# dtarb/TauDEM

Measured on AMD Instinct MI355X. Metric: Mcells/s (PitRemove->D8FlowDir->AreaD8 pipeline), higher is better.
Workload: dtype f32

## Files before the change

### taudem_amd/csrc/d8flowdir.hip

```cpp
#include <cstring>

#include "context.hpp"
#include "device_common.hpp"
#include "flats.hpp"

namespace {

using namespace tdxk;

constexpr int SLOPE_ROWS = 16;

constexpr int SLOPE_COLS = 62;
using flatmask_t = uint32_t;
template <int SLOPE_SEG>
__global__ __launch_bounds__(256) void d8_slope_kernel(const float* __restrict__ Z, int nx, int ny, int y_own0, int y_own1, float nodata,
                                                       const double* __restrict__ fact, int16_t* __restrict__ P,
                                                       float* __restrict__ SD8, flatmask_t* __restrict__ flatbits, int nbx, int xmap) {
    using tilek::lane_left;
    using tilek::lane_right;
    const int bx = tdxk::xcd_block_x(nbx, xmap);
    if (bx < 0) return;
    const int lx = threadIdx.x & 63;
    const int x = bx * SLOPE_COLS - 1 + lx;
    const int band = __builtin_amdgcn_readfirstlane(int(blockIdx.y) * 4 + int(threadIdx.x >> 6));
// ... 76 lines not shown
    for (unsigned b0 = 0; b0 < nblocks; b0 += 1024) {
        const unsigned i = b0 + threadIdx.x;
        const unsigned long long own = i < nblocks ? blocksum[i] : 0u;
        unsigned long long v = own;
#pragma unroll
        for (int off = 1; off < 64; off <<= 1) {
            const unsigned long long t = __shfl_up(v, off, 64);
            if (int(threadIdx.x & 63) >= off) v += t;
        }
        if ((threadIdx.x & 63) == 63) sw[threadIdx.x >> 6] = v;
        __syncthreads();
        unsigned long long wave_off = carry;
        for (unsigned w = 0; w < (threadIdx.x >> 6); w++) wave_off += sw[w];
        if (i < nblocks) blocksum[i] = unsigned(wave_off + v - own);
        __syncthreads();
        if (threadIdx.x == 1023) carry = wave_off + v;
        __syncthreads();
    }
    if (threadIdx.x == 0) *total = carry;
}
__global__ __launch_bounds__(256) void flat_list_kernel(const flatmask_t* __restrict__ bits, size_t nmasks, int nx, int y_own0, int seg, const unsigned* __restrict__ blockoff,
                                                        uint32_t* __restrict__ list) {
    constexpr int NCH = FLATQ_PER_BLOCK / 256;
    const size_t base = size_t(blockIdx.x) * FLATQ_PER_BLOCK + threadIdx.x;
    const int lane = int(threadIdx.x & 63), w = int(threadIdx.x >> 6);
    unsigned mk[NCH];
    __shared__ unsigned scnt[NCH][4];
#pragma unroll
    for (int i = 0; i < NCH; i++) {
        const size_t m = base + size_t(i) * 256;
        mk[i] = m < nmasks ? bits[m] : 0u;
        unsigned c = unsigned(__popc(mk[i]));
#pragma unroll
        for (int off = 32; off >= 1; off >>= 1) c += __shfl_xor(c, off, 64);
        if (lane == 0) scnt[i][w] = c;
    }
    __syncthreads();
    const unsigned long long below = (1ull << lane) - 1ull;
#pragma unroll
    for (int i = 0; i < NCH; i++) {
        unsigned any = mk[i];
#pragma unroll
        for (int off = 32; off >= 1; off >>= 1) any |= __shfl_xor(any, off, 64);
        if (!any) continue;
        unsigned pos = blockoff[blockIdx.x];
        for (int j = 0; j < i; j++) pos += scnt[j][0] + scnt[j][1] + scnt[j][2] + scnt[j][3];
        for (int u = 0; u < w; u++) pos += scnt[i][u];
        const size_t m = base + size_t(i) * 256, mc = m < nmasks ? m : nmasks - 1;
        const unsigned band = unsigned(mc / size_t(nx)), x = unsigned(mc - size_t(band) * size_t(nx));
        const size_t c0 = size_t(y_own0 + int(band) * seg) * size_t(nx) + size_t(x);
        for (unsigned rows = any; rows; rows &= rows - 1u) {
            const int r = __ffs(int(rows)) - 1;
            const bool mine = (mk[i] >> r) & 1u;
            const unsigned long long b = __ballot(mine);
            if (mine) list[pos + unsigned(__popcll(b & below))] = uint32_t(c0 + size_t(r) * size_t(nx));
            pos += unsigned(__popcll(b));
        }
    }
}

__device__ __forceinline__ bool dont_cross_d8(const int16_t* __restrict__ P, size_t c, int nx, int k) {
    switch (k) {
        case 2: return P[c + 1] == 4 || P[c - nx] == 8;
        case 4: return P[c - nx] == 6 || P[c - 1] == 2;
        case 6: return P[c + nx] == 4 || P[c - 1] == 8;
        case 8: return P[c + 1] == 6 || P[c + nx] == 2;
        default: return false;
    }
}

struct D8Codes {
    using Raw = int;
    const int16_t* P;
    __device__ __forceinline__ int load(size_t o) const { return P[o]; }
    static __device__ __forceinline__ unsigned onehot(int p) { return (1u << min(unsigned(p), 31u)) & 0x1FFu; }
};

struct D8Traits {
    const int16_t* P;
    __device__ __forceinline__ bool dont_cross(size_t c, int nx, int k) const { return dont_cross_d8(P, c, nx, k); }
    __device__ __forceinline__ bool has_direction(size_t n) const { const int16_t v = P[n]; return v > 0 && v < 9; }
};

template <class LV>
__global__ __launch_bounds__(256) void d8_setflow2_kernel(const float* __restrict__ Z, int nx, const double* __restrict__ fact,
                                                          const uint32_t* __restrict__ list, unsigned long long nq,
                                                          const LV* __restrict__ lvl, const LV* __restrict__ rq,
                                                          FlatLevels fl, int16_t* __restrict__ P) {
    const unsigned long long q = (unsigned long long)blockIdx.x * 256 + threadIdx.x;
    if (q >= nq) return;
    const size_t c = list[q];
    const int y = int(c / size_t(nx));
    const double* f = fact + size_t(y) * 9;
    const int e2c = int(flat_elev2<LV>(lvl[c], rq[c], fl));
    const float z0 = Z[c];
    float smax = 0.f;
    int16_t dir = P[c];
    const int order[8] = {1, 3, 5, 7, 2, 4, 6, 8};
    for (int o = 0; o < 8; o++) {
        const int k = order[o];
        const size_t n = size_t(ptrdiff_t(c) + ptrdiff_t(d2(k)) * nx + d1(k));
        if (rq[n] > 0) {
            const int e2n = int(flat_elev2<LV>(lvl[n], rq[n], fl));
            const float slope = (float)(f[k] * (double)(e2c - e2n));
            if (slope > smax) { dir = int16_t(k); smax = slope; }
        } else {
            const float ed = z0 - Z[n];
            if (ed >= 0) { dir = int16_t(k); break; }
        }
    }
    P[c] = dir;
}

__global__ __launch_bounds__(256) void d8_recollect_kernel(const int16_t* __restrict__ P, const uint32_t* __restrict__ list,
                                                           unsigned long long nq, uint32_t* __restrict__ out,
                                                           unsigned long long* __restrict__ counter) {
    const unsigned long long q0 = ((unsigned long long)blockIdx.x * 256 + threadIdx.x) * 8;
    uint32_t keep[8];
    unsigned cnt = 0;
#pragma unroll
    for (int i = 0; i < 8; i++) {
        const unsigned long long q = q0 + (unsigned long long)i;
        if (q < nq) {
            const uint32_t c = list[q];
            if (P[c] == 0) keep[cnt++] = c;
        }
    }
    unsigned long long pos = block_reserve(cnt, counter);
    for (unsigned i = 0; i < cnt; i++) out[pos + i] = keep[i];
}

template <class LV>
__global__ __launch_bounds__(256) void d8_mark_pits_kernel(const uint32_t* __restrict__ list, unsigned long long nq,
                                                           const LV* __restrict__ lvl, int16_t* __restrict__ P) {
    const unsigned long long q = (unsigned long long)blockIdx.x * 256 + threadIdx.x;
    if (q >= nq) return;
    const size_t c = list[q];
    if (lvl[c] == 0) P[c] = TDX_P_NODATA;
}

constexpr int SF2_COLS = 62;
template <class LV>
__global__ __launch_bounds__(256) void d8_setflow2_stream_kernel(const float* __restrict__ Z, int nx, int ny, int y_own0, int y_own1,
                                                                 const double* __restrict__ fact, const LV* __restrict__ lvl,
                                                                 const LV* __restrict__ rq, FlatLevels fl, int16_t* __restrict__ P,
                                                                 uint32_t* __restrict__ qnext, unsigned long long* __restrict__ counter, int nbx, int xmap,
                                                                 LV* __restrict__ lvl_next, LV* __restrict__ rq_next) {
    using tilek::lane_left;
    using tilek::lane_right;
    const int bx = tdxk::xcd_block_x(nbx, xmap);
    if (bx < 0) return;
    const int lx = threadIdx.x & 63;
    const int x = bx * SF2_COLS - 1 + lx;
    const int ybase = __builtin_amdgcn_readfirstlane(y_own0 + blockIdx.y * (4 * SLOPE_ROWS) + (threadIdx.x >> 6) * SLOPE_ROWS);
    const bool mine = lx >= 1 && lx <= SF2_COLS && x < nx;
    const int xc = x < 0 ? 0 : (x >= nx ? nx - 1 : x);
    int16_t p[SLOPE_ROWS];
#pragma unroll
    for (int r = 0; r < SLOPE_ROWS; r++) {
        const int y = ybase + r, yc = y >= ny ? ny - 1 : y;
        p[r] = P[size_t(yc) * size_t(nx) + size_t(xc)];
    }
    unsigned flat = 0;
    unsigned rows0 = 0;
#pragma unroll
    for (int r = 0; r < SLOPE_ROWS; r++) {
        const bool f0 = mine && ybase + r < y_own1 && p[r] == 0;
        if (f0) flat |= 1u << r;
        if (__ballot(f0) != 0ull) rows0 |= 1u << r;
    }
    unsigned keep = 0;
    if (rows0) {
        const unsigned need = rows0 | (rows0 << 1) | (rows0 << 2);
        float z[SLOPE_ROWS + 2];
        int e2[SLOPE_ROWS + 2], rr[SLOPE_ROWS + 2];
#pragma unroll
        for (int j = 0; j < SLOPE_ROWS + 2; j++) {
            z[j] = 0.f; e2[j] = -1; rr[j] = -1;
            if ((need >> j) & 1u) {
                const int y = ybase - 1 + j, yc = y < 0 ? 0 : (y >= ny ? ny - 1 : y);
                const size_t o = size_t(yc) * size_t(nx) + size_t(xc);
                z[j] = Z[o]; e2[j] = lvl[o]; rr[j] = rq[o];
            }
        }
        unsigned pit = 0;
#pragma unroll
        for (int j = 0; j < SLOPE_ROWS + 2; j++) {
            if (e2[j] == 0) pit |= 1u << j;
            e2[j] = int(flat_elev2<LV>(e2[j], rr[j], fl));
        }
#pragma unroll
        for (int r = 0; r < SLOPE_ROWS; r++) {
            if (!((rows0 >> r) & 1u)) continue;
            const int y = ybase + r;
            const float zk[9] = {0.f, lane_right(z[r + 1], 0.f), lane_right(z[r], 0.f), z[r], lane_left(z[r], 0.f), lane_left(z[r + 1], 0.f),
                                 lane_left(z[r + 2], 0.f), z[r + 2], lane_right(z[r + 2], 0.f)};
            const int rk[9] = {0, lane_right(rr[r + 1], -1), lane_right(rr[r], -1), rr[r], lane_left(rr[r], -1), lane_left(rr[r + 1], -1),
                               lane_left(rr[r + 2], -1), rr[r + 2], lane_right(rr[r + 2], -1)};
            const int ek[9] = {0, lane_right(e2[r + 1], 0), lane_right(e2[r], 0), e2[r], lane_left(e2[r], 0), lane_left(e2[r + 1], 0),
                               lane_left(e2[r + 2], 0), e2[r + 2], lane_right(e2[r + 2], 0)};
            if ((flat >> r) & 1u) {
                const double* f = fact + size_t(y) * 9;
                const int e2c = e2[r + 1];
                const float z0 = z[r + 1];
                float smax = 0.f;
                int16_t dir = (fl.has_pits && ((pit >> (r + 1)) & 1u)) ? TDX_P_NODATA : int16_t(0);
                bool done = false;
#define TDX_SF2(K)                                                                     \
    if (!done) {                                                                        \
        const float slope = (float)(f[K] * (double)(e2c - ek[K]));                      \
        const bool marked = rk[K] > 0;                                                  \
        const bool take = marked && slope > smax;                                       \
        const bool stop = !marked && z0 - zk[K] >= 0;                                   \
        dir = (take || stop) ? int16_t(K) : dir;                                        \
        smax = take ? slope : smax;                                                     \
        done = stop;                                                                    \
    }
                TDX_SF2(1) TDX_SF2(3) TDX_SF2(5) TDX_SF2(7) TDX_SF2(2) TDX_SF2(4) TDX_SF2(6) TDX_SF2(8)
#undef TDX_SF2
                P[size_t(y) * size_t(nx) + size_t(x)] = dir;
                if (dir == 0) keep |= 1u << r;
            }
        }
    }
    if (lvl_next != nullptr) {
#pragma unroll
        for (int r = 0; r < SLOPE_ROWS; r++) {
            if (mine && ybase + r < y_own1) {
                const size_t idx = size_t(ybase + r) * size_t(nx) + size_t(x);
                const LV m = ((keep >> r) & 1u) ? LV(0) : LV(-1);
                lvl_next[idx] = m;
                rq_next[idx] = m;
            }
        }
    }
    const unsigned long long pos = block_reserve(unsigned(__popc(keep)), counter);
    const unsigned long long wbase = (unsigned long long)(unsigned(__builtin_amdgcn_readfirstlane(int(unsigned(pos))))) |
                                     ((unsigned long long)(unsigned(__builtin_amdgcn_readfirstlane(int(unsigned(pos >> 32))))) << 32);
    const unsigned long long below = (1ull << lx) - 1ull;
    unsigned rowoff = 0;
#pragma unroll
    for (int r = 0; r < SLOPE_ROWS; r++) {
        const unsigned long long b = __ballot((keep >> r) & 1u);
        if ((keep >> r) & 1u) qnext[wbase + rowoff + unsigned(__popcll(b & below))] = uint32_t(size_t(ybase + r) * size_t(nx) + size_t(x));
        rowoff += unsigned(__popcll(b));
    }
}

}

int tdx_build_fact_table(tdx_context* ctx, int64_t ny, const double* dxc, const double* dyc, double** d_fact_out) {
    static const int hd1[9] = {0, 1, 1, 0, -1, -1, -1, 0, 1};
    static const int hd2[9] = {0, 0, -1, -1, -1, 0, 1, 1, 1};
    const size_t rows = size_t(ny);
    if (ctx->fact_dxc.size() == rows && ctx->fact_dyc.size() == rows && memcmp(ctx->fact_dxc.data(), dxc, rows * 8) == 0 &&
        memcmp(ctx->fact_dyc.data(), dyc, rows * 8) == 0) {
        *d_fact_out = static_cast<double*>(ctx->scratch(TDX_S_FACT, rows * 9 * sizeof(double)));
        return *d_fact_out ? TDX_OK : TDX_ERR_NOMEM;
    }
    ctx->fact_dxc.clear(); ctx->fact_dyc.clear();
    std::vector<double> fact(rows * 9, 0.0);
    for (int64_t m = 0; m < ny; m++)
        for (int k = 1; k <= 8; k++)
            fact[size_t(m) * 9 + size_t(k)] = (double)(1. / sqrt(hd1[k] * hd1[k] * dxc[m] * dxc[m] + hd2[k] * hd2[k] * dyc[m] * dyc[m]));
    double* d_fact = static_cast<double*>(ctx->scratch(TDX_S_FACT, fact.size() * sizeof(double)));
    if (!d_fact) return TDX_ERR_NOMEM;
    TDX_HIP_CHECK(ctx, hipMemcpyAsync(d_fact, fact.data(), fact.size() * sizeof(double), hipMemcpyHostToDevice, ctx->stream));
    TDX_HIP_CHECK(ctx, hipStreamSynchronize(ctx->stream));
    ctx->fact_dxc.assign(dxc, dxc + rows);
    ctx->fact_dyc.assign(dyc, dyc + rows);
    *d_fact_out = d_fact;
    return TDX_OK;
}

template <class LV>
static int d8flowdir_levels(tdx_context* ctx, const Strip& st, float* d_fel, float fel_nodata, const double* dxc, const double* dyc, int16_t* d_p,
                          float* d_sd8, tdx_stats* stats) {
    TDX_HIP_CHECK(ctx, hipSetDevice(ctx->device));
    hipStream_t s = ctx->stream;
    const int inx = st.nx;
    const size_t n = size_t(st.nx) * size_t(st.ny_arr);
    double* d_fact = nullptr;
    int rc = tdx_build_fact_table(ctx, st.ny_arr, dxc, dyc, &d_fact);
    if (rc != TDX_OK) return rc;
    unsigned long long* d_cnt = reinterpret_cast<unsigned long long*>(ctx->d_mail);
    LV* lvl = static_cast<LV*>(ctx->scratch(TDX_S_A, n * sizeof(LV)));
    LV* rq = static_cast<LV*>(ctx->scratch(TDX_S_B, n * sizeof(LV)));
    uint32_t* qlist = static_cast<uint32_t*>(ctx->scratch(TDX_S_C, n * 4));
    if (!lvl || !rq || !qlist) return TDX_ERR_NOMEM;

    ctx->begin_call(stats);
    strip_mark(ctx, st, "d8flowdir");
    ctx->phase = "slope pass";
    rc = strip_exchange<float>(ctx, st, d_fel, fel_nodata);
    if (rc != TDX_OK) return rc;
    TDX_HIP_CHECK(ctx, hipMemsetAsync(d_cnt, 0, 8 * sizeof(unsigned long long), s));
    static const int seg = (getenv("TDX_SLOPE_SEG") && atoi(getenv("TDX_SLOPE_SEG")) == 16) ? 16 : 32;
    const int nband = ((st.y1 - st.y0 + 4 * seg - 1) / (4 * seg)) * 4;
    const size_t nmasks = size_t(nband) * size_t(inx);
    const unsigned nqblocks = unsigned((nmasks + FLATQ_PER_BLOCK - 1) / FLATQ_PER_BLOCK);
    flatmask_t* flatbits = static_cast<flatmask_t*>(ctx->scratch(TDX_S_N, nmasks * sizeof(flatmask_t)));
    unsigned* blocksum = static_cast<unsigned*>(ctx->scratch(TDX_S_O, size_t(nqblocks) * 4));
    if (!flatbits || !blocksum) return TDX_ERR_NOMEM;
    {
        TdxSpan sp(ctx, TDX_K_STENCIL);
        const int nbx = (inx + SLOPE_COLS - 1) / SLOPE_COLS, xmap = tdx_xcd_map() ? 1 : 0;
        dim3 grid(tdx_xcd_grid_x(unsigned(nbx)), unsigned(nband / 4));
        if (seg == 16) hipLaunchKernelGGL(d8_slope_kernel<16>, grid, dim3(256), 0, s, d_fel, inx, st.ny_arr, st.y0, st.y1, fel_nodata, d_fact, d_p, d_sd8, flatbits, nbx, xmap);
        else hipLaunchKernelGGL(d8_slope_kernel<32>, grid, dim3(256), 0, s, d_fel, inx, st.ny_arr, st.y0, st.y1, fel_nodata, d_fact, d_p, d_sd8, flatbits, nbx, xmap);
        if (stats) stats->launches[TDX_K_STENCIL]++;
    }
    {
        TdxSpan sp(ctx, TDX_K_MISC);
        hipLaunchKernelGGL(flat_count_kernel, dim3(nqblocks), dim3(256), 0, s, flatbits, nmasks, blocksum);
        hipLaunchKernelGGL(flat_scan_kernel, dim3(1), dim3(1024), 0, s, blocksum, nqblocks, d_cnt);
    }
    TDX_HIP_CHECK(ctx, hipMemcpyAsync(ctx->h_mail, d_cnt, sizeof(unsigned long long), hipMemcpyDeviceToHost, s));
    TDX_HIP_CHECK(ctx, hipStreamSynchronize(s));
    unsigned long long nq = ctx->h_mail[0];
    int64_t total = int64_t(nq);
    rc = strip_allreduce(ctx, st, &total, 1, TDX_OP_SUM);
    if (rc != TDX_OK) return rc;
    if (stats) { stats->flats_initial = total; stats->flats_left = total; }

    const bool force_list = getenv("TDX_FLATS_LIST") != nullptr;
    const bool have_list = force_list || nq <= n / 16;
    if (total > 0 && nq > 0 && have_list) {
        TdxSpan sp(ctx, TDX_K_MISC);
        hipLaunchKernelGGL(flat_list_kernel, dim3(nqblocks), dim3(256), 0, s, flatbits, nmasks, inx, st.y0, seg, blocksum, qlist);
    }
    if (total > 0) {
        rc = strip_exchange<int16_t>(ctx, st, d_p, TDX_P_NODATA);
        if (rc != TDX_OK) return rc;
        uint32_t* qnext = static_cast<uint32_t*>(ctx->scratch(TDX_S_D, size_t(nq) * 4));
        if (!qnext) return TDX_ERR_NOMEM;
        float* zwork = nullptr;
        const float* zcur = d_fel;
        FlatBuffersT<LV> fbuf{lvl, rq};

        int64_t last = total;
        const int64_t total0 = total;
        bool sparse = false;
        unsigned long long nq_old = 0;
        bool old_list_valid = false;
        LV *lvl_next = nullptr, *rq_next = nullptr;
        bool markers_ready = false;
        for (int iteration = 1;; iteration++) {
            const FlatPhases& ph = flat_phases(iteration);
            ctx->phase = ph.classify;
            FlatLevels fl;
            D8Traits tr{d_p};
            const float* zc = zcur;
            const StreamClassifyFn classify = [&](const tilek::TileGeom& g, uint8_t* fmask, uint8_t* rmask, uint32_t* tile_flags, uint8_t* tile_masked, uint8_t* notfull) {
                const int nbx = (st.nx + flatk::CLS_COLS - 1) / flatk::CLS_COLS;
                const dim3 grid(tdx_xcd_grid_x(unsigned(nbx)), (st.y1 - st.y0 + 4 * flatk::CLS_ROWS - 1) / (4 * flatk::CLS_ROWS));
                hipLaunchKernelGGL((flatk::classify_stream_kernel<LV, D8Codes>), grid, dim3(256), 0, s, zc, D8Codes{d_p}, st.nx, st.ny_arr, st.y0, st.y1, g.tiles_x, lvl, rq, fmask,
                                   rmask, tile_flags, tile_masked, nbx, tdx_xcd_map() ? 1 : 0, notfull);
            };
            if (sparse && markers_ready) {
                std::swap(lvl, lvl_next);
                std::swap(rq, rq_next);
                fbuf = FlatBuffersT<LV>{lvl, rq};
                rc = strip_exchange<LV>(ctx, st, lvl, LV(-1));
                if (rc != TDX_OK) return rc;
                rc = strip_exchange<LV>(ctx, st, rq, LV(-1));
                if (rc != TDX_OK) return rc;
            } else if (sparse) {
                rc = old_list_valid ? flats_reset_markers_after(ctx, st, qnext, nq_old, qlist, nq, lvl, rq) : flats_reset_markers(ctx, st, qlist, nq, lvl, rq);
                if (rc != TDX_OK) return rc;
            }
            markers_ready = false;
            rc = flats_bfs<D8Traits, LV>(ctx, tr, zcur, st, (nq_old == 0 && !have_list) ? nullptr : qlist, nq, fbuf, &fl, stats, sparse ? nullptr : &classify, iteration);
            if (rc != TDX_OK) return rc;
            ctx->phase = ph.directions;
            {
                TdxSpan sp(ctx, TDX_K_FLATDIR);
                unsigned long long* d_next = d_cnt + 4;
                if (nq > n / 32) {
                    const int nbx = (st.nx + SF2_COLS - 1) / SF2_COLS;
                    const dim3 grid(tdx_xcd_grid_x(unsigned(nbx)), (st.y1 - st.y0 + 4 * SLOPE_ROWS - 1) / (4 * SLOPE_ROWS));
                    static const bool no_next = getenv("TDX_FLATS_NO_NEXT_MARKERS") != nullptr;
                    if (!no_next && !lvl_next) {
                        lvl_next = static_cast<LV*>(ctx->scratch(TDX_S_P, n * sizeof(LV)));
                        rq_next = static_cast<LV*>(ctx->scratch(TDX_S_R, n * sizeof(LV)));
                        if (!lvl_next || !rq_next) return TDX_ERR_NOMEM;
                    }
                    hipLaunchKernelGGL((d8_setflow2_stream_kernel<LV>), grid, dim3(256), 0, s, zcur, inx, st.ny_arr, st.y0, st.y1, d_fact, lvl, rq, fl, d_p, qnext,
                                       d_next, nbx, tdx_xcd_map() ? 1 : 0, lvl_next, rq_next);
                    markers_ready = lvl_next != nullptr;
                } else if (nq) {
                    if (fl.has_pits)
                        hipLaunchKernelGGL((d8_mark_pits_kernel<LV>), dim3(tdx_blocks_for(nq, 256)), dim3(256), 0, s, qlist, nq, lvl, d_p);
                    hipLaunchKernelGGL((d8_setflow2_kernel<LV>), dim3(tdx_blocks_for(nq, 256)), dim3(256), 0, s, zcur, inx, d_fact, qlist, nq, lvl, rq, fl, d_p);
                    hipLaunchKernelGGL(d8_recollect_kernel, dim3(tdx_blocks_for(nq, 2048)), dim3(256), 0, s, d_p, qlist, nq, qnext, d_next);
                }
                TDX_HIP_CHECK(ctx, hipMemcpyAsync(ctx->h_mail, d_next, sizeof(unsigned long long), hipMemcpyDeviceToHost, s));
                TDX_HIP_CHECK(ctx, hipStreamSynchronize(s));
                if (stats) stats->launches[TDX_K_FLATDIR] += 2 + (fl.has_pits ? 1 : 0);
            }
            const unsigned long long nleft = ctx->h_mail[0];
            total = int64_t(nleft);
            rc = strip_allreduce(ctx, st, &total, 1, TDX_OP_SUM);
            if (rc != TDX_OK) return rc;
            rc = strip_exchange<int16_t>(ctx, st, d_p, TDX_P_NODATA);
            if (rc != TDX_OK) return rc;
            if (stats) { stats->flat_iterations++; stats->flats_left = total; }
            if (!(total > 0 && total < last)) break;
            ctx->phase = ph.next;
            if (!zwork) {
                zwork = static_cast<float*>(ctx->scratch(TDX_S_I, n * 4));
                if (!zwork) return TDX_ERR_NOMEM;
            }
            static const bool no_sparse = getenv("TDX_FLATS_DENSE") != nullptr;
            sparse = !no_sparse && (total * 8 <= total0 || total <= (int64_t(1) << 20));
            rc = sparse ? flats_overwrite_elevation_sparse(ctx, inx, qnext, nleft, lvl, rq, fl, zwork) : flats_overwrite_elevation(ctx, n, lvl, rq, fl, zwork);
            if (rc != TDX_OK) return rc;
            zcur = zwork;
            old_list_valid = nq_old != 0 || have_list;
            nq_old = nq;
            std::swap(qlist, qnext);
            nq = nleft;
            last = total;
        }
    }
    TDX_HIP_CHECK(ctx, hipGetLastError());
    ctx->end_call();
    return TDX_OK;
}

static int d8flowdir_impl(tdx_context* ctx, const Strip& st, float* d_fel, float fel_nodata, const double* dxc, const double* dyc, int16_t* d_p,
                          float* d_sd8, tdx_stats* stats) {
    int rc = getenv("TDX_LEVELS_INT32") ? TDX_FLATS_TOO_DEEP : d8flowdir_levels<int16_t>(ctx, st, d_fel, fel_nodata, dxc, dyc, d_p, d_sd8, stats);
    if (rc == TDX_FLATS_TOO_DEEP) rc = d8flowdir_levels<int32_t>(ctx, st, d_fel, fel_nodata, dxc, dyc, d_p, d_sd8, stats);
    return rc;
}

static int d8flowdir_check(tdx_context* ctx, const void* fel, const void* p, const void* dxc, const void* dyc, int64_t nx, int64_t ny, int64_t halo, const char* who) {
    if (!ctx || !fel || !p || !dxc || !dyc || nx <= 0 || ny <= 0) return tdx_fail(ctx, TDX_ERR_ARG, who);
    return too_big(nx, ny + halo) ? tdx_fail(ctx, TDX_ERR_ARG, "raster larger than 2^32 cells per device strip") : TDX_OK;
}

extern "C" int tdx_d8flowdir_dev(tdx_context* ctx, const float* d_fel, int64_t nx, int64_t ny, float fel_nodata,
                                 const double* dxc, const double* dyc, int16_t* d_p, float* d_sd8, tdx_stats* stats) {
    if (int rc = d8flowdir_check(ctx, d_fel, d_p, dxc, dyc, nx, ny, 0, "tdx_d8flowdir_dev: bad argument")) return rc;
    return d8flowdir_impl(ctx, strip_single(int(nx), int(ny)), const_cast<float*>(d_fel), fel_nodata, dxc, dyc, d_p, d_sd8, stats);
}

extern "C" int tdx_d8flowdir_strip(tdx_context* ctx, const tdx_comm* comm, float* d_fel, int64_t nx, int64_t ny_local, float fel_nodata,
                                   const double* dxc, const double* dyc, int16_t* d_p, float* d_sd8, tdx_stats* stats) {
    if (int rc = d8flowdir_check(ctx, d_fel, d_p, dxc, dyc, nx, ny_local, 2, "tdx_d8flowdir_strip: bad argument")) return rc;
    return d8flowdir_impl(ctx, strip_from_comm(comm, int(nx), int(ny_local)), d_fel, fel_nodata, dxc, dyc, d_p, d_sd8, stats);
}

extern "C" int tdx_d8flowdir(tdx_context* ctx, const float* fel, int64_t nx, int64_t ny, float fel_nodata,
                             const double* dxc, const double* dyc, int16_t* p, float* sd8, tdx_stats* stats) {
    if (!ctx || !fel || !p || nx <= 0 || ny <= 0) return tdx_fail(ctx, TDX_ERR_ARG, "tdx_d8flowdir: bad argument");
    HostCall h(ctx, nx, ny);
    float* d_z = h.in(TDX_S_IO0, fel);
    int16_t* d_p = h.out(TDX_S_IO1, p);
    float* d_s = h.out(TDX_S_IO2, sd8);
    if (h.error) return h.error;
    return h.finish(tdx_d8flowdir_dev(ctx, d_z, nx, ny, fel_nodata, dxc, dyc, d_p, d_s, stats));
}
```

### taudem_amd/csrc/dinfflowdir.hip

```cpp
#include "context.hpp"
#include "device_common.hpp"
#include "flats.hpp"

namespace {
using namespace tdxk;

#define TDX_PI 3.14159265359

__host__ __device__ constexpr int fI1(int K) { return int((0x1a505u >> (2 * K)) & 3u) - 1; }
__host__ __device__ constexpr int fI2(int K) { return int((0x2a801u >> (2 * K)) & 3u) - 1; }
__host__ __device__ constexpr int fJ1(int K) { return int((0x25059u >> (2 * K)) & 3u) - 1; }
__host__ __device__ constexpr int fJ2(int K) { return int((0x28029u >> (2 * K)) & 3u) - 1; }
__host__ __device__ constexpr bool fID1_is1(int K) { return ((0x132u >> K) & 1u) != 0u; }
__host__ __device__ constexpr double fANGC(int K) { return double(K / 2); }
__host__ __device__ constexpr double fANGF(int K) { return (K & 1) ? 1.0 : -1.0; }
__device__ __forceinline__ double fANGC_rt(int K) { return double(K >> 1); }
__device__ __forceinline__ double fANGF_rt(int K) { return (K & 1) ? 1.0 : -1.0; }
static_assert(fI1(3) == -1 && fI2(5) == 1 && fJ1(4) == -1 && fJ2(8) == 1 && fID1_is1(1) && !fID1_is1(2) && fID1_is1(8), "facet tables");

struct RowGeom { double dx, dy, dd, ad12, ad21; };

__device__ __forceinline__ void vslope(double E0, double E1, double E2, double D1, double D2, double DD, double AD, double& S, double& A) {
    double S1 = 0, S2 = 0;
    if (D1 != 0) S1 = (E0 - E1) / D1;
    if (D2 != 0) S2 = (E1 - E2) / D2;
    if (S2 == 0 && S1 == 0) A = 0;
    else A = atan2(S2, S1);
    if (A < 0.) { A = 0.; S = S1; }
    else if (A > AD) { A = AD; S = (E0 - E2) / DD; }
    else S = sqrt(S1 * S1 + S2 * S2);
}

__device__ __forceinline__ void facet_geom(const RowGeom& g, int K, double& D1, double& D2, double& AD) {
    const bool one = fID1_is1(K);
    D1 = one ? g.dx : g.dy;
    D2 = one ? g.dy : g.dx;
    AD = one ? g.ad12 : g.ad21;
}

template <class T>
__device__ __forceinline__ T sel4(int i, T a0, T a1, T a2, T a3) { return i == 0 ? a0 : (i == 1 ? a1 : (i == 2 ? a2 : a3)); }
__device__ __forceinline__ int facet_cardinal(int K) { return (K & 7) >> 1; }
__device__ __forceinline__ int facet_diagonal(int K) { return (K - 1) >> 1; }

__device__ __forceinline__ double vslope_s(double E0, double E1, double E2, double D1, double D2, double DD, double AD, int* kind, double* s1o, double* s2o) {
    const double S1 = (E0 - E1) / D1, S2 = (E1 - E2) / D2;
    *s1o = S1; *s2o = S2;
    int kd;
    if (S2 == 0 && S1 == 0) kd = 2;
    else if (S2 < 0) kd = 0;
    else if (S2 == 0) kd = S1 > 0 ? 2 : 1;
    else if (S1 <= 0) kd = 1;
    else {
        const double l = S2 * D1, r = S1 * D2;
        if (fabs(l - r) > 1e-9 * (l + r)) kd = l > r ? 1 : 2;
        else kd = atan2(S2, S1) > atan2(D2, D1) ? 1 : 2;
    }
    *kind = kd;
    if (kd == 0) return S1;
    if (kd == 1) return (E0 - E2) / DD;
    return sqrt(S1 * S1 + S2 * S2);
}

constexpr int DSLOPE_ROWS = 16;
__global__ __launch_bounds__(256) void dinf_slope_kernel(const float* __restrict__ Z, int nx, int ny, int y_own0, int y_own1, float nodata,
                                                         const RowGeom* __restrict__ geom, float* __restrict__ ANG,
                                                         float* __restrict__ SLP, unsigned long long* __restrict__ nflat) {
    const int x = blockIdx.x * 64 + (threadIdx.x & 63);
    const int ybase = y_own0 + blockIdx.y * (4 * DSLOPE_ROWS) + (threadIdx.x >> 6) * DSLOPE_ROWS;
    const bool colok = x < nx;
    const int xc = colok ? x : nx - 1, xm = xc > 0 ? xc - 1 : xc, xp = xc < nx - 1 ? xc + 1 : xc;
    auto ldrow = [&](int y, float& a, float& b, float& c) {
        if (y >= 0 && y < ny) {
            const float* r = Z + size_t(y) * size_t(nx);
            a = r[xm]; b = r[xc]; c = r[xp];
        } else { a = b = c = nodata; }
    };
    float n0, n1, n2, c0, c1, c2, s0, s1, s2;
    ldrow(ybase - 1, n0, n1, n2);
    ldrow(ybase, c0, c1, c2);
    unsigned nfl = 0;
#pragma unroll
// ... 36 lines not shown
                }
            }
            ANG[idx] = ang;
            SLP[idx] = slp;
        }
        n0 = c0; n1 = c1; n2 = c2;
        c0 = s0; c1 = s1; c2 = s2;
    }
    (void)block_reserve(nfl, nflat);
}


struct DinfTraits {
    const float* ANG;
    __device__ __forceinline__ bool dont_cross(size_t c, int nx, int k) const {
        switch (k) {
            case 2: return ANG[c + 1] == 4 || ANG[c - nx] == 8;
            case 4: return ANG[c - nx] == 6 || ANG[c - 1] == 2;
            case 6: return ANG[c + nx] == 4 || ANG[c - 1] == 8;
            case 8: return ANG[c + 1] == 6 || ANG[c + nx] == 2;
            default: return false;
        }
    }
    __device__ __forceinline__ bool has_direction(size_t n) const { return ANG[n] >= 0.0f; }
};

__device__ __forceinline__ bool dinf_is_flat(float a) { return !is_nodata_f(a, TDX_ANG_NODATA) && a < 0.0f; }

struct DinfCodes {
    using Raw = float;
    const float* ANG;
    __device__ __forceinline__ float load(size_t o) const { return ANG[o]; }
    static __device__ __forceinline__ unsigned onehot(float a) {
        if (is_nodata_f(a, TDX_ANG_NODATA)) return 0u;
        if (a < 0.0f) return 1u;
        return a == 2.0f ? 1u << 2 : (a == 4.0f ? 1u << 4 : (a == 6.0f ? 1u << 6 : (a == 8.0f ? 1u << 8 : 1u << 1)));
    }
};

template <class LV>
__global__ __launch_bounds__(256) void dinf_collect_flats_kernel(const float* __restrict__ ANG, size_t first, size_t n, LV* __restrict__ lvl,
                                                                 LV* __restrict__ rq, uint32_t* __restrict__ list,
                                                                 unsigned long long* __restrict__ counter) {
    const size_t c0 = first + (size_t(blockIdx.x) * 256 + threadIdx.x) * 8;
    unsigned mask = 0;
    float a[8];
    const bool whole = c0 + 8 <= n && (reinterpret_cast<uintptr_t>(ANG + c0) & 15u) == 0;
    if (whole) {
        const float4 a0 = *reinterpret_cast<const float4*>(ANG + c0), a1 = *reinterpret_cast<const float4*>(ANG + c0 + 4);
        a[0] = a0.x; a[1] = a0.y; a[2] = a0.z; a[3] = a0.w; a[4] = a1.x; a[5] = a1.y; a[6] = a1.z; a[7] = a1.w;
    } else {
#pragma unroll
        for (int i = 0; i < 8; i++) a[i] = c0 + i < n ? ANG[c0 + i] : TDX_ANG_NODATA;
    }
#pragma unroll
    for (int i = 0; i < 8; i++)
        if (c0 + i < n && dinf_is_flat(a[i])) mask |= 1u << i;
    if (sizeof(LV) == 2 && c0 + 8 <= n && ((reinterpret_cast<uintptr_t>(lvl + c0) | reinterpret_cast<uintptr_t>(rq + c0)) & 15u) == 0) {
        unsigned w[4];
#pragma unroll
        for (int j = 0; j < 4; j++) w[j] = (((mask >> (2 * j)) & 1u) ? 0u : 0xFFFFu) | (((mask >> (2 * j + 1)) & 1u) ? 0u : 0xFFFF0000u);
        *reinterpret_cast<uint4*>(lvl + c0) = make_uint4(w[0], w[1], w[2], w[3]);
        *reinterpret_cast<uint4*>(rq + c0) = make_uint4(w[0], w[1], w[2], w[3]);
    } else {
#pragma unroll
        for (int i = 0; i < 8; i++)
            if (c0 + i < n) { const LV m = ((mask >> i) & 1u) ? LV(0) : LV(-1); lvl[c0 + i] = m; rq[c0 + i] = m; }
    }
    unsigned long long pos = block_reserve(unsigned(__popc(mask)), counter);
#pragma unroll
    for (int i = 0; i < 8; i++)
        if (mask & (1u << i)) list[pos++] = uint32_t(c0 + size_t(i));
}

template <class LV>
__global__ __launch_bounds__(256) void dinf_mark_pits_kernel(const uint32_t* __restrict__ list, unsigned long long nq,
                                                             const LV* __restrict__ lvl, float* __restrict__ ANG) {
    const unsigned long long q = (unsigned long long)blockIdx.x * 256 + threadIdx.x;
    if (q >= nq) return;
    const size_t c = list[q];
    if (lvl[c] == 0) ANG[c] = TDX_ANG_NODATA;
}

template <class LV>
__global__ __launch_bounds__(256) void dinf_set2flat_kernel(const float* __restrict__ Z, int nx, const RowGeom* __restrict__ geom,
                                                            const uint32_t* __restrict__ list, unsigned long long nq,
                                                            const LV* __restrict__ lvl, const LV* __restrict__ rq,
                                                            FlatLevels fl, float* __restrict__ ANG) {
    const unsigned long long q = (unsigned long long)blockIdx.x * 256 + threadIdx.x;
    if (q >= nq) return;
    const size_t c0 = list[q];
    const int y = int(c0 / size_t(nx));
    float zw[9];
    LV lw[9], rw[9];
#pragma unroll
    for (int i = 0; i < 9; i++) {
        const size_t n = size_t(ptrdiff_t(c0) + ptrdiff_t(i / 3 - 1) * nx + (i % 3 - 1));
        zw[i] = Z[n]; lw[i] = lvl[n]; rw[i] = rq[n];
    }
    const float ang0 = ANG[c0];
    const RowGeom g = geom[y];
    int e2w[9];
#pragma unroll
    for (int i = 0; i < 9; i++) e2w[i] = int(flat_elev2<LV>(lw[i], rw[i], fl));
    double SMAX = 0.0;
    int KD = 0, KINDW = 0;
    double S1W = 0., S2W = 0.;
    bool diagOutFound = false, done = false;
    const double a = (double)zw[4];
    const int a1 = e2w[4];
#pragma unroll 1
    for (int K = 1; K <= 8 && !done; K++) {
        const int j1 = facet_cardinal(K), j2 = facet_diagonal(K);
        const float zb = sel4(j1, zw[5], zw[1], zw[3], zw[7]), zc = sel4(j2, zw[2], zw[0], zw[6], zw[8]);
        const bool in1 = sel4(j1, rw[5], rw[1], rw[3], rw[7]) > 0, in2 = sel4(j2, rw[2], rw[0], rw[6], rw[8]) > 0;
        const int l1 = sel4(j1, e2w[5], e2w[1], e2w[3], e2w[7]), l2 = sel4(j2, e2w[2], e2w[0], e2w[6], e2w[8]);
        const double b = (double)zb, cc = (double)zc;
        if (!in1 && in2 && a >= b) { KD = K; KINDW = 0; done = true; continue; }
        if (in1 && !in2 && a >= cc) { if (!diagOutFound) { KD = K; KINDW = 1; diagOutFound = true; } continue; }
        const bool real = !in1 && !in2;
        const double E0 = real ? a : (double)a1;
        const double E1 = real ? b : (double)(in1 ? l1 : (a1 > l2 ? a1 : l2));
        const double E2 = real ? cc : (double)(in2 ? l2 : (a1 > l1 ? a1 : l1));
        double D1, D2, AD, sa, sb;
        facet_geom(g, K, D1, D2, AD);
        int kind;
        const double S = vslope_s(E0, E1, E2, D1, D2, g.dd, AD, &kind, &sa, &sb);
        if (real) {
            if (S >= 0.0) {
                if (b > a) { if (!diagOutFound) { diagOutFound = true; KD = K; KINDW = kind; S1W = sa; S2W = sb; } }
                else { KD = K; KINDW = kind; S1W = sa; S2W = sb; done = true; }
            }
        } else if (S > SMAX) { SMAX = S; KD = K; KINDW = kind; S1W = sa; S2W = sb; }
    }
    float ang = ang0;
    if (!is_nodata_f(ang, TDX_ANG_NODATA)) ang = -1.f;
    if (KD > 0) {
        double D1, D2, AD;
        facet_geom(g, KD, D1, D2, AD);
        const double AKD = KINDW == 0 ? 0. : (KINDW == 1 ? AD : ((S2W == 0 && S1W == 0) ? 0. : atan2(S2W, S1W)));
        const float t = (float)(fANGC(KD) * (TDX_PI / 2) + fANGF(KD) * AKD);
        if (t >= 0.0f) ang = t;
    }
    ANG[c0] = ang;
}

__global__ __launch_bounds__(256) void dinf_recollect_kernel(const float* __restrict__ ANG, const uint32_t* __restrict__ list,
                                                             unsigned long long nq, uint32_t* __restrict__ out,
                                                             unsigned long long* __restrict__ counter) {
    const unsigned long long q0 = ((unsigned long long)blockIdx.x * 256 + threadIdx.x) * 8;
    uint32_t keep[8];
    unsigned cnt = 0;
#pragma unroll
    for (int i = 0; i < 8; i++) {
        const unsigned long long q = q0 + (unsigned long long)i;
        if (q < nq) {
            const uint32_t c = list[q];
            if (dinf_is_flat(ANG[c])) keep[cnt++] = c;
        }
    }
    unsigned long long pos = block_reserve(cnt, counter);
    for (unsigned i = 0; i < cnt; i++) out[pos + i] = keep[i];
}

}

template <class LV>
static int dinfflowdir_levels(tdx_context* ctx, const Strip& st, float* d_fel, float fel_nodata, const double* dxc, const double* dyc, float* d_ang,
                            float* d_slp, tdx_stats* stats) {
    TDX_HIP_CHECK(ctx, hipSetDevice(ctx->device));
    hipStream_t s = ctx->stream;
    const int inx = st.nx, iny = st.ny_arr;
    const size_t n = size_t(inx) * size_t(iny);
    std::vector<RowGeom> geom;
    geom.resize(size_t(iny));
    for (int j = 0; j < iny; j++) {
        RowGeom g;
        g.dx = dxc[j]; g.dy = dyc[j];
        g.dd = sqrt(dxc[j] * dxc[j] + dyc[j] * dyc[j]);
        g.ad12 = atan2(dyc[j], dxc[j]);
        g.ad21 = atan2(dxc[j], dyc[j]);
        geom[size_t(j)] = g;
    }
    RowGeom* d_geom = static_cast<RowGeom*>(ctx->scratch(TDX_S_J, geom.size() * sizeof(RowGeom)));
    if (!d_geom) return TDX_ERR_NOMEM;
    TDX_HIP_CHECK(ctx, hipMemcpyAsync(d_geom, geom.data(), geom.size() * sizeof(RowGeom), hipMemcpyHostToDevice, s));
    TDX_HIP_CHECK(ctx, hipStreamSynchronize(s));
    unsigned long long* d_cnt = reinterpret_cast<unsigned long long*>(ctx->d_mail);

    ctx->begin_call(stats);
    strip_mark(ctx, st, "dinfflowdir");
    ctx->phase = "slope pass";
    int rc = strip_exchange<float>(ctx, st, d_fel, fel_nodata);
    if (rc != TDX_OK) return rc;
    TDX_HIP_CHECK(ctx, hipMemsetAsync(d_cnt, 0, 8 * sizeof(unsigned long long), s));
    {
        TdxSpan sp(ctx, TDX_K_STENCIL);
        dim3 grid((inx + 63) / 64, (st.y1 - st.y0 + 4 * DSLOPE_ROWS - 1) / (4 * DSLOPE_ROWS));
        hipLaunchKernelGGL(dinf_slope_kernel, grid, dim3(256), 0, s, d_fel, inx, iny, st.y0, st.y1, fel_nodata, d_geom, d_ang, d_slp, d_cnt);
        if (stats) stats->launches[TDX_K_STENCIL]++;
    }
    TDX_HIP_CHECK(ctx, hipMemcpyAsync(ctx->h_mail, d_cnt, sizeof(unsigned long long), hipMemcpyDeviceToHost, s));
    TDX_HIP_CHECK(ctx, hipStreamSynchronize(s));
    unsigned long long nq = ctx->h_mail[0];
    int64_t total = int64_t(nq);
    rc = strip_allreduce(ctx, st, &total, 1, TDX_OP_SUM);
    if (rc != TDX_OK) return rc;
    if (stats) { stats->flats_initial = total; stats->flats_left = total; }

    if (total > 0) {
        LV* lvl = static_cast<LV*>(ctx->scratch(TDX_S_A, n * sizeof(LV)));
        LV* rq = static_cast<LV*>(ctx->scratch(TDX_S_B, n * sizeof(LV)));
        uint32_t* qlist = static_cast<uint32_t*>(ctx->scratch(TDX_S_C, size_t(nq) * 4));
        uint32_t* qnext = static_cast<uint32_t*>(ctx->scratch(TDX_S_D, size_t(nq) * 4));
        if (!lvl || !rq || !qlist || !qnext) return TDX_ERR_NOMEM;
        float* zwork = nullptr;
        const float* zcur = d_fel;
        FlatBuffersT<LV> fbuf{lvl, rq};
        rc = strip_exchange<float>(ctx, st, d_ang, TDX_ANG_NODATA);
        if (rc != TDX_OK) return rc;
        TDX_HIP_CHECK(ctx, hipMemsetAsync(d_cnt, 0, 8 * sizeof(unsigned long long), s));
        const size_t own_first = size_t(st.y0) * size_t(inx), own_end = size_t(st.y1) * size_t(inx);
        hipLaunchKernelGGL((dinf_collect_flats_kernel<LV>), dim3(tdx_blocks_for(own_end - own_first, 2048)), dim3(256), 0, s, d_ang, own_first, own_end, lvl, rq,
                           qlist, d_cnt);
        rc = strip_exchange<LV>(ctx, st, lvl, LV(-1));
        if (rc != TDX_OK) return rc;
        rc = strip_exchange<LV>(ctx, st, rq, LV(-1));
        if (rc != TDX_OK) return rc;
        int64_t last = total;
        bool first = true;
        unsigned long long nq_old = 0;
        for (int iteration = 1;; iteration++) {
            const FlatPhases& ph = flat_phases(iteration);
            ctx->phase = ph.classify;
            if (!first) { rc = flats_reset_markers_after(ctx, st, qnext, nq_old, qlist, nq, lvl, rq); if (rc != TDX_OK) return rc; }
            first = false;
            FlatLevels fl;
            DinfTraits tr{d_ang};
            const float* zc = zcur;
            const StreamClassifyFn classify = [&](const tilek::TileGeom& g, uint8_t* fmask, uint8_t* rmask, uint32_t* tile_flags, uint8_t* tile_masked, uint8_t* notfull) {
                const int nbx = (st.nx + flatk::CLS_COLS - 1) / flatk::CLS_COLS;
                const dim3 grid(tdx_xcd_grid_x(unsigned(nbx)), (st.y1 - st.y0 + 4 * flatk::CLS_ROWS - 1) / (4 * flatk::CLS_ROWS));
                hipLaunchKernelGGL((flatk::classify_stream_kernel<LV, DinfCodes>), grid, dim3(256), 0, s, zc, DinfCodes{d_ang}, st.nx, st.ny_arr, st.y0, st.y1, g.tiles_x, lvl, rq,
                                   fmask, rmask, tile_flags, tile_masked, nbx, tdx_xcd_map() ? 1 : 0, notfull);
            };
            const bool force_list = getenv("TDX_FLATS_LIST") != nullptr;
            const bool dense = !force_list && nq > n / 16;
            rc = flats_bfs<DinfTraits, LV>(ctx, tr, zcur, st, qlist, nq, fbuf, &fl, stats, dense ? &classify : nullptr, iteration);
            if (rc != TDX_OK) return rc;
            ctx->phase = ph.directions;
            {
                TdxSpan sp(ctx, TDX_K_FLATDIR);
                unsigned long long* d_next = d_cnt + 4;
                if (nq) {
                    if (fl.has_pits)
                        hipLaunchKernelGGL((dinf_mark_pits_kernel<LV>), dim3(tdx_blocks_for(nq, 256)), dim3(256), 0, s, qlist, nq, lvl, d_ang);
                    hipLaunchKernelGGL((dinf_set2flat_kernel<LV>), dim3(tdx_blocks_for(nq, 256)), dim3(256), 0, s, zcur, inx, d_geom, qlist, nq, lvl, rq, fl, d_ang);
                    hipLaunchKernelGGL(dinf_recollect_kernel, dim3(tdx_blocks_for(nq, 2048)), dim3(256), 0, s, d_ang, qlist, nq, qnext, d_next);
                }
                TDX_HIP_CHECK(ctx, hipMemcpyAsync(ctx->h_mail, d_next, sizeof(unsigned long long), hipMemcpyDeviceToHost, s));
                TDX_HIP_CHECK(ctx, hipStreamSynchronize(s));
                if (stats) stats->launches[TDX_K_FLATDIR] += 2 + (fl.has_pits ? 1 : 0);
            }
            const unsigned long long nleft = ctx->h_mail[0];
            total = int64_t(nleft);
            rc = strip_allreduce(ctx, st, &total, 1, TDX_OP_SUM);
            if (rc != TDX_OK) return rc;
            rc = strip_exchange<float>(ctx, st, d_ang, TDX_ANG_NODATA);
            if (rc != TDX_OK) return rc;
            if (stats) { stats->flat_iterations++; stats->flats_left = total; }
            if (!(total > 0 && total < last)) break;
            ctx->phase = ph.next;
            if (!zwork) { zwork = static_cast<float*>(ctx->scratch(TDX_S_I, n * 4)); if (!zwork) return TDX_ERR_NOMEM; }
            rc = nleft <= n / 32 ? flats_overwrite_elevation_sparse(ctx, inx, qnext, nleft, lvl, rq, fl, zwork) : flats_overwrite_elevation(ctx, n, lvl, rq, fl, zwork);
            if (rc != TDX_OK) return rc;
            zcur = zwork;
            nq_old = nq;
            std::swap(qlist, qnext);
            nq = nleft; last = total;
        }
    }
    TDX_HIP_CHECK(ctx, hipGetLastError());
    ctx->end_call();
    return TDX_OK;
}

static int dinfflowdir_impl(tdx_context* ctx, const Strip& st, float* d_fel, float fel_nodata, const double* dxc, const double* dyc, float* d_ang,
                            float* d_slp, tdx_stats* stats) {
    int rc = getenv("TDX_LEVELS_INT32") ? TDX_FLATS_TOO_DEEP : dinfflowdir_levels<int16_t>(ctx, st, d_fel, fel_nodata, dxc, dyc, d_ang, d_slp, stats);
    if (rc == TDX_FLATS_TOO_DEEP) rc = dinfflowdir_levels<int32_t>(ctx, st, d_fel, fel_nodata, dxc, dyc, d_ang, d_slp, stats);
    return rc;
}

static int dinfflowdir_check(tdx_context* ctx, const void* fel, const void* ang, const void* slp, const void* dxc, const void* dyc, int64_t nx, int64_t ny,
                             int64_t halo, const char* who) {
    if (!ctx || !fel || !ang || !slp || !dxc || !dyc || nx <= 0 || ny <= 0) return tdx_fail(ctx, TDX_ERR_ARG, who);
    return too_big(nx, ny + halo) ? tdx_fail(ctx, TDX_ERR_ARG, "raster larger than 2^32 cells per device strip") : TDX_OK;
}

extern "C" int tdx_dinfflowdir_dev(tdx_context* ctx, const float* d_fel, int64_t nx, int64_t ny, float fel_nodata,
                                   const double* dxc, const double* dyc, float* d_ang, float* d_slp, tdx_stats* stats) {
    if (int rc = dinfflowdir_check(ctx, d_fel, d_ang, d_slp, dxc, dyc, nx, ny, 0, "tdx_dinfflowdir_dev: bad argument")) return rc;
    return dinfflowdir_impl(ctx, strip_single(int(nx), int(ny)), const_cast<float*>(d_fel), fel_nodata, dxc, dyc, d_ang, d_slp, stats);
}

extern "C" int tdx_dinfflowdir_strip(tdx_context* ctx, const tdx_comm* comm, float* d_fel, int64_t nx, int64_t ny_local, float fel_nodata,
                                     const double* dxc, const double* dyc, float* d_ang, float* d_slp, tdx_stats* stats) {
    if (int rc = dinfflowdir_check(ctx, d_fel, d_ang, d_slp, dxc, dyc, nx, ny_local, 2, "tdx_dinfflowdir_strip: bad argument")) return rc;
    return dinfflowdir_impl(ctx, strip_from_comm(comm, int(nx), int(ny_local)), d_fel, fel_nodata, dxc, dyc, d_ang, d_slp, stats);
}

extern "C" int tdx_dinfflowdir(tdx_context* ctx, const float* fel, int64_t nx, int64_t ny, float fel_nodata,
                               const double* dxc, const double* dyc, float* ang, float* slp, tdx_stats* stats) {
    if (!ctx || !fel || !ang || !slp || nx <= 0 || ny <= 0) return tdx_fail(ctx, TDX_ERR_ARG, "tdx_dinfflowdir: bad argument");
    HostCall h(ctx, nx, ny);
    float* d_z = h.in(TDX_S_IO0, fel);
    float* d_a = h.out(TDX_S_IO1, ang);
    float* d_s = h.out(TDX_S_IO2, slp);
    if (h.error) return h.error;
    return h.finish(tdx_dinfflowdir_dev(ctx, d_z, nx, ny, fel_nodata, dxc, dyc, d_a, d_s, stats));
}
```

Before: 14110.

## Fuse flat pit-marking, set-flow and recollect into single kernels; fold elevation overwrite

In both the D8 and Dinf flat resolution loops, the separate mark-pits, set-flow and recollect kernels are merged into one kernel per iteration. That kernel computes the initial direction inline, writes the result, and appends still-flat cells to the next queue through a block reservation. The dense D8 streaming set-flow kernel now also writes the overwritten flat elevation for kept cells and their neighbours, so the separate sparse overwrite pass can be skipped. The aim is fewer launches and fewer passes over memory per flat iteration, at the cost of more complex kernels and new environment switches for falling back to the old path.

```diff
diff --git a/taudem_amd/csrc/d8flowdir.hip b/taudem_amd/csrc/d8flowdir.hip
--- a/taudem_amd/csrc/d8flowdir.hip
+++ b/taudem_amd/csrc/d8flowdir.hip
@@ -182,34 +182,45 @@
     __device__ __forceinline__ bool has_direction(size_t n) const { const int16_t v = P[n]; return v > 0 && v < 9; }
 };
 
-template <class LV>
+template <class LV, bool FUSED>
 __global__ __launch_bounds__(256) void d8_setflow2_kernel(const float* __restrict__ Z, int nx, const double* __restrict__ fact,
                                                           const uint32_t* __restrict__ list, unsigned long long nq,
                                                           const LV* __restrict__ lvl, const LV* __restrict__ rq,
-                                                          FlatLevels fl, int16_t* __restrict__ P) {
+                                                          FlatLevels fl, int16_t* __restrict__ P, uint32_t* __restrict__ qnext,
+                                                          unsigned long long* __restrict__ counter) {
     const unsigned long long q = (unsigned long long)blockIdx.x * 256 + threadIdx.x;
-    if (q >= nq) return;
-    const size_t c = list[q];
-    const int y = int(c / size_t(nx));
-    const double* f = fact + size_t(y) * 9;
-    const int e2c = int(flat_elev2<LV>(lvl[c], rq[c], fl));
-    const float z0 = Z[c];
-    float smax = 0.f;
-    int16_t dir = P[c];
-    const int order[8] = {1, 3, 5, 7, 2, 4, 6, 8};
-    for (int o = 0; o < 8; o++) {
-        const int k = order[o];
-        const size_t n = size_t(ptrdiff_t(c) + ptrdiff_t(d2(k)) * nx + d1(k));
-        if (rq[n] > 0) {
-            const int e2n = int(flat_elev2<LV>(lvl[n], rq[n], fl));
-            const float slope = (float)(f[k] * (double)(e2c - e2n));
-            if (slope > smax) { dir = int16_t(k); smax = slope; }
-        } else {
-            const float ed = z0 - Z[n];
-            if (ed >= 0) { dir = int16_t(k); break; }
-        }
-    }
-    P[c] = dir;
+    const bool live = q < nq;
+    size_t c = 0;
+    int16_t dir = 1;
+    if (live) {
+        c = list[q];
+        const int y = int(c / size_t(nx));
+        const double* f = fact + size_t(y) * 9;
+        const int l0 = lvl[c];
+        const int e2c = int(flat_elev2<LV>(l0, rq[c], fl));
+        const float z0 = Z[c];
+        float smax = 0.f;
+        dir = FUSED ? ((fl.has_pits && l0 == 0) ? TDX_P_NODATA : int16_t(0)) : P[c];
+        const int order[8] = {1, 3, 5, 7, 2, 4, 6, 8};
+        for (int o = 0; o < 8; o++) {
+            const int k = order[o];
+            const size_t n = size_t(ptrdiff_t(c) + ptrdiff_t(d2(k)) * nx + d1(k));
+            if (rq[n] > 0) {
+                const int e2n = int(flat_elev2<LV>(lvl[n], rq[n], fl));
+                const float slope = (float)(f[k] * (double)(e2c - e2n));
+                if (slope > smax) { dir = int16_t(k); smax = slope; }
+            } else {
+                const float ed = z0 - Z[n];
+                if (ed >= 0) { dir = int16_t(k); break; }
+            }
+        }
+        P[c] = dir;
+    }
+    if (FUSED) {
+        const bool still_flat = live && dir == 0;
+        const unsigned long long pos = block_reserve(still_flat ? 1u : 0u, counter);
+        if (still_flat) qnext[pos] = uint32_t(c);
+    }
 }
 
 __global__ __launch_bounds__(256) void d8_recollect_kernel(const int16_t* __restrict__ P, const uint32_t* __restrict__ list,
@@ -245,7 +256,7 @@
                                                                  const double* __restrict__ fact, const LV* __restrict__ lvl,
                                                                  const LV* __restrict__ rq, FlatLevels fl, int16_t* __restrict__ P,
                                                                  uint32_t* __restrict__ qnext, unsigned long long* __restrict__ counter, int nbx, int xmap,
-                                                                 LV* __restrict__ lvl_next, LV* __restrict__ rq_next) {
+                                                                 LV* __restrict__ lvl_next, LV* __restrict__ rq_next, float* __restrict__ Znext) {
     using tilek::lane_left;
     using tilek::lane_right;
     const int bx = tdxk::xcd_block_x(nbx, xmap);
@@ -345,6 +356,17 @@
         if ((keep >> r) & 1u) qnext[wbase + rowoff + unsigned(__popcll(b & below))] = uint32_t(size_t(ybase + r) * size_t(nx) + size_t(x));
         rowoff += unsigned(__popcll(b));
     }
+    if (Znext != nullptr && __ballot(keep != 0u) != 0ull) {
+        const unsigned kc = keep | lane_left(keep, 0u) | lane_right(keep, 0u);
+        const unsigned wm = (x >= 0 && x < nx) ? (kc | (kc << 1) | (kc << 2)) : 0u;
+#pragma unroll
+        for (int j = 0; j < SLOPE_ROWS + 2; j++) {
+            if ((wm >> j) & 1u) {
+                const size_t o = size_t(ybase - 1 + j) * size_t(nx) + size_t(x);
+                Znext[o] = (float)flat_elev2<LV>(lvl[o], rq[o], fl);
+            }
+        }
+    }
 }
 
 }
@@ -445,6 +467,11 @@
         bool old_list_valid = false;
         LV *lvl_next = nullptr, *rq_next = nullptr;
         bool markers_ready = false;
+        bool elev_ready = false;
+        const char* sw_over = getenv("TDX_FLATS_OVERWRITE");
+        const char* sw_setf = getenv("TDX_FLATS_SETFLOW");
+        const bool overwrite_pass = sw_over && strcmp(sw_over, "pass") == 0;
+        const bool setflow_split = sw_setf && strcmp(sw_setf, "split") == 0;
         for (int iteration = 1;; iteration++) {
             const FlatPhases& ph = flat_phases(iteration);
             ctx->phase = ph.classify;
@@ -476,6 +503,8 @@
             {
                 TdxSpan sp(ctx, TDX_K_FLATDIR);
                 unsigned long long* d_next = d_cnt + 4;
+                int nlaunch = 0;
+                elev_ready = false;
                 if (nq > n / 32) {
                     const int nbx = (st.nx + SF2_COLS - 1) / SF2_COLS;
                     const dim3 grid(tdx_xcd_grid_x(unsigned(nbx)), (st.y1 - st.y0 + 4 * SLOPE_ROWS - 1) / (4 * SLOPE_ROWS));
@@ -485,18 +514,32 @@
                         rq_next = static_cast<LV*>(ctx->scratch(TDX_S_R, n * sizeof(LV)));
                         if (!lvl_next || !rq_next) return TDX_ERR_NOMEM;
                     }
+                    float* znext = nullptr;
+                    if (!overwrite_pass && zcur == d_fel) {
+                        if (!zwork) zwork = static_cast<float*>(ctx->scratch(TDX_S_I, n * 4));
+                        if (!zwork) return TDX_ERR_NOMEM;
+                        znext = zwork;
+                    }
                     hipLaunchKernelGGL((d8_setflow2_stream_kernel<LV>), grid, dim3(256), 0, s, zcur, inx, st.ny_arr, st.y0, st.y1, d_fact, lvl, rq, fl, d_p, qnext,
-                                       d_next, nbx, tdx_xcd_map() ? 1 : 0, lvl_next, rq_next);
+                                       d_next, nbx, tdx_xcd_map() ? 1 : 0, lvl_next, rq_next, znext);
                     markers_ready = lvl_next != nullptr;
-                } else if (nq) {
+                    elev_ready = znext != nullptr;
+                    nlaunch = 1;
+                } else if (nq && setflow_split) {
                     if (fl.has_pits)
                         hipLaunchKernelGGL((d8_mark_pits_kernel<LV>), dim3(tdx_blocks_for(nq, 256)), dim3(256), 0, s, qlist, nq, lvl, d_p);
-                    hipLaunchKernelGGL((d8_setflow2_kernel<LV>), dim3(tdx_blocks_for(nq, 256)), dim3(256), 0, s, zcur, inx, d_fact, qlist, nq, lvl, rq, fl, d_p);
+                    hipLaunchKernelGGL((d8_setflow2_kernel<LV, false>), dim3(tdx_blocks_for(nq, 256)), dim3(256), 0, s, zcur, inx, d_fact, qlist, nq, lvl, rq, fl, d_p,
+                                       static_cast<uint32_t*>(nullptr), static_cast<unsigned long long*>(nullptr));
                     hipLaunchKernelGGL(d8_recollect_kernel, dim3(tdx_blocks_for(nq, 2048)), dim3(256), 0, s, d_p, qlist, nq, qnext, d_next);
+                    nlaunch = 2 + (fl.has_pits ? 1 : 0);
+                } else if (nq) {
+                    hipLaunchKernelGGL((d8_setflow2_kernel<LV, true>), dim3(tdx_blocks_for(nq, 256)), dim3(256), 0, s, zcur, inx, d_fact, qlist, nq, lvl, rq, fl, d_p, qnext,
+                                       d_next);
+                    nlaunch = 1;
                 }
                 TDX_HIP_CHECK(ctx, hipMemcpyAsync(ctx->h_mail, d_next, sizeof(unsigned long long), hipMemcpyDeviceToHost, s));
                 TDX_HIP_CHECK(ctx, hipStreamSynchronize(s));
-                if (stats) stats->launches[TDX_K_FLATDIR] += 2 + (fl.has_pits ? 1 : 0);
+                if (stats) stats->launches[TDX_K_FLATDIR] += nlaunch;
             }
             const unsigned long long nleft = ctx->h_mail[0];
             total = int64_t(nleft);
@@ -511,9 +554,9 @@
                 zwork = static_cast<float*>(ctx->scratch(TDX_S_I, n * 4));
                 if (!zwork) return TDX_ERR_NOMEM;
             }
-            static const bool no_sparse = getenv("TDX_FLATS_DENSE") != nullptr;
+            const bool no_sparse = getenv("TDX_FLATS_DENSE") != nullptr;
             sparse = !no_sparse && (total * 8 <= total0 || total <= (int64_t(1) << 20));
-            rc = sparse ? flats_overwrite_elevation_sparse(ctx, inx, qnext, nleft, lvl, rq, fl, zwork) : flats_overwrite_elevation(ctx, n, lvl, rq, fl, zwork);
+            rc = !sparse ? flats_overwrite_elevation(ctx, n, lvl, rq, fl, zwork) : (elev_ready ? TDX_OK : flats_overwrite_elevation_sparse(ctx, inx, qnext, nleft, lvl, rq, fl, zwork));
             if (rc != TDX_OK) return rc;
             zcur = zwork;
             old_list_valid = nq_old != 0 || have_list;
diff --git a/taudem_amd/csrc/dinfflowdir.hip b/taudem_amd/csrc/dinfflowdir.hip
--- a/taudem_amd/csrc/dinfflowdir.hip
+++ b/taudem_amd/csrc/dinfflowdir.hip
@@ -1,3 +1,5 @@
+#include <cstring>
+
 #include "context.hpp"
 #include "device_common.hpp"
 #include "flats.hpp"
@@ -200,14 +202,9 @@
     if (lvl[c] == 0) ANG[c] = TDX_ANG_NODATA;
 }
 
-template <class LV>
-__global__ __launch_bounds__(256) void dinf_set2flat_kernel(const float* __restrict__ Z, int nx, const RowGeom* __restrict__ geom,
-                                                            const uint32_t* __restrict__ list, unsigned long long nq,
-                                                            const LV* __restrict__ lvl, const LV* __restrict__ rq,
-                                                            FlatLevels fl, float* __restrict__ ANG) {
-    const unsigned long long q = (unsigned long long)blockIdx.x * 256 + threadIdx.x;
-    if (q >= nq) return;
-    const size_t c0 = list[q];
+template <class LV, bool FUSED>
+__device__ __forceinline__ float dinf_set2flat_cell(const float* __restrict__ Z, int nx, const RowGeom* __restrict__ geom, size_t c0,
+                                                    const LV* __restrict__ lvl, const LV* __restrict__ rq, FlatLevels fl, const float* __restrict__ ANG) {
     const int y = int(c0 / size_t(nx));
     float zw[9];
     LV lw[9], rw[9];
@@ -216,7 +213,7 @@
         const size_t n = size_t(ptrdiff_t(c0) + ptrdiff_t(i / 3 - 1) * nx + (i % 3 - 1));
         zw[i] = Z[n]; lw[i] = lvl[n]; rw[i] = rq[n];
     }
-    const float ang0 = ANG[c0];
+    const float ang0 = FUSED ? ((fl.has_pits && lw[4] == 0) ? TDX_ANG_NODATA : -1.f) : ANG[c0];
     const RowGeom g = geom[y];
     int e2w[9];
 #pragma unroll
@@ -260,7 +257,29 @@
         const float t = (float)(fANGC(KD) * (TDX_PI / 2) + fANGF(KD) * AKD);
         if (t >= 0.0f) ang = t;
     }
-    ANG[c0] = ang;
+    return ang;
+}
+
+template <class LV, bool FUSED>
+__global__ __launch_bounds__(256) void dinf_set2flat_kernel(const float* __restrict__ Z, int nx, const RowGeom* __restrict__ geom,
+                                                            const uint32_t* __restrict__ list, unsigned long long nq,
+                                                            const LV* __restrict__ lvl, const LV* __restrict__ rq,
+                                                            FlatLevels fl, float* __restrict__ ANG, uint32_t* __restrict__ qnext,
+                                                            unsigned long long* __restrict__ counter) {
+    const unsigned long long q = (unsigned long long)blockIdx.x * 256 + threadIdx.x;
+    const bool live = q < nq;
+    size_t c0 = 0;
+    bool still_flat = false;
+    if (live) {
+        c0 = list[q];
+        const float ang = dinf_set2flat_cell<LV, FUSED>(Z, nx, geom, c0, lvl, rq, fl, ANG);
+        ANG[c0] = ang;
+        still_flat = dinf_is_flat(ang);
+    }
+    if (FUSED) {
+        const unsigned long long pos = block_reserve(still_flat ? 1u : 0u, counter);
+        if (still_flat) qnext[pos] = uint32_t(c0);
+    }
 }
 
 __global__ __launch_bounds__(256) void dinf_recollect_kernel(const float* __restrict__ ANG, const uint32_t* __restrict__ list,
@@ -370,15 +389,23 @@
             {
                 TdxSpan sp(ctx, TDX_K_FLATDIR);
                 unsigned long long* d_next = d_cnt + 4;
-                if (nq) {
+                const char* sw_setf = getenv("TDX_FLATS_SETFLOW");
+                int nlaunch = 0;
+                if (nq && sw_setf && strcmp(sw_setf, "split") == 0) {
                     if (fl.has_pits)
                         hipLaunchKernelGGL((dinf_mark_pits_kernel<LV>), dim3(tdx_blocks_for(nq, 256)), dim3(256), 0, s, qlist, nq, lvl, d_ang);
-                    hipLaunchKernelGGL((dinf_set2flat_kernel<LV>), dim3(tdx_blocks_for(nq, 256)), dim3(256), 0, s, zcur, inx, d_geom, qlist, nq, lvl, rq, fl, d_ang);
+                    hipLaunchKernelGGL((dinf_set2flat_kernel<LV, false>), dim3(tdx_blocks_for(nq, 256)), dim3(256), 0, s, zcur, inx, d_geom, qlist, nq, lvl, rq, fl, d_ang,
+                                       static_cast<uint32_t*>(nullptr), static_cast<unsigned long long*>(nullptr));
                     hipLaunchKernelGGL(dinf_recollect_kernel, dim3(tdx_blocks_for(nq, 2048)), dim3(256), 0, s, d_ang, qlist, nq, qnext, d_next);
+                    nlaunch = 2 + (fl.has_pits ? 1 : 0);
+                } else if (nq) {
+                    hipLaunchKernelGGL((dinf_set2flat_kernel<LV, true>), dim3(tdx_blocks_for(nq, 256)), dim3(256), 0, s, zcur, inx, d_geom, qlist, nq, lvl, rq, fl, d_ang, qnext,
+                                       d_next);
+                    nlaunch = 1;
                 }
                 TDX_HIP_CHECK(ctx, hipMemcpyAsync(ctx->h_mail, d_next, sizeof(unsigned long long), hipMemcpyDeviceToHost, s));
                 TDX_HIP_CHECK(ctx, hipStreamSynchronize(s));
-                if (stats) stats->launches[TDX_K_FLATDIR] += 2 + (fl.has_pits ? 1 : 0);
+                if (stats) stats->launches[TDX_K_FLATDIR] += nlaunch;
             }
             const unsigned long long nleft = ctx->h_mail[0];
             total = int64_t(nleft);
```

New measurement: 14230 (median of 6 runs). No clear change (+0.8%).
